# MarineRoboticsGroup/score

Hardware: AMD Instinct MI355X
Metric: socp_iters_per_sec (higher is better)
Workload: dtype f64; 1 GPU; BASELINE configs[3]: manhattan RA-SLAM, 20 robots x 1000 poses, 4 beacons, SOCP relaxation, 1 trial(s)/GPU, ADMM loop alone (polish off) to eps 1e-07; n=146995, m=80979, nnz_P=946147, parallelism=independent x1

## Files before the change

score_amd/csrc/score_hip.hip:

```cpp
#include <hip/hip_runtime.h>
#include <sched.h>
#include <sys/prctl.h>
#include <time.h>
#include <hip/hip_ext.h>

#include <cstdio>
#include <cstring>
#include <malloc.h>
#include <mutex>
#include <string>
#include <memory>
#include <optional>
#include <vector>

#include "score_driver.hpp"
#include <future>
#include "score_assemble.hpp"
#include "score_gn_kernels.hpp"
#include "score_round.hpp"
#include "score_kernels.hpp"
#include "score_polish.hpp"
#include "score_polish_device.hpp"
#include "score_setup_device.hpp"
#include "score_prec_wave.hpp"
// ... 766 lines not shown
    DevBuf<double> cone_vals;
    DevBuf<int32_t> node_col, diag_cols, prec_part_ptr;
    DevBuf<PrecWork> prec_work, factor_work;
    DevBuf<int64_t> q_entpart;
    int64_t q_ent_max = 0;
    static constexpr int64_t kHelpEntries = (int64_t)kPrecThreads * kPrecChunk;
    int n_help = 0;
    DevBuf<int32_t> vb_first, vb_end, vb_prob;
    int n_vblocks = 0;
    DevBuf<double> xtu, xy, s, r, z, p, p2, w, kx, step;
    DevBuf<double> pw_part, rz_part0, rz_part1, rz_meas0, rz_meas1, pres_part, dres_part;
    struct GenSource {
        const int32_t* rel_base; const int32_t* rel_to; const double* rel_t; const double* rel_R; const double* rel_kappa; const double* rel_tau;
        const int32_t* rng_a; const int32_t* rng_b; const double* rng_dist; const double* rng_prec;
    };
    const GenSource* gen_src = nullptr;
    int n_join_items = 0, n_join_chains = 0, n_join_seps = 0;
    DevBuf<JoinChain> join_jc;
    DevBuf<JoinItem> join_items;
    DevBuf<int32_t> join_sep_col, join_sep_diag, join_pcol, join_pprev, join_zero;
    DevBuf<double> join_rhs, join_tmp_p, join_tmp_rz, join_zb;
    DevBuf<int32_t> deep_map;
    bool prec_reg = false;
    size_t prec_reg_lds = 0;
    PolishData Q;
    std::future<void> polish_build;
    bool polish_on_device = false;
    bool derive_ag = false;
    int64_t hm_nnz = 0;
    CsrBufs Hm;
    struct PrecSet {
        const CsrBufs& mat;
        const BandBufs& band;
        const DevBuf<PrecWork>& fac_work;
        PrecSet(const CsrBufs& m, const BandBufs& b, const DevBuf<PrecWork>& fw) : mat(m), band(b), fac_work(fw) {}
        DevBuf<ChainDesc> chains;
        DevBuf<ChainLevelDesc> levels;
        DevBuf<PrecRecord> rec;
        DevBuf<int64_t> fac_range;
        DevBuf<double> fac, dinv;
        DevBuf<float> fac32;
        DevBuf<float> deep;
        size_t fac_doubles = 0;
        int64_t deep_floats = 0;
        bool use_fac32 = false;
        bool use_owner = false;
        DevBuf<int32_t> posd, poss, diagpos;
        DevBuf<int32_t> blk_part;
        int blocks() const { return band.on ? band.nblocks : mat.nblocks; }
        DevBuf<double> join_W, join_data;
        DevBuf<int32_t> join_posd, join_poss;
        bool link_on = false;
        DevBuf<int32_t> link_pcol, link_pshift, link_pos, link_status;
        DevBuf<double> link_Qt, link_Zr;
    };
    PrecSet pset[2] = {{K, Kb, factor_work}, {Hm, Hb, prec_work}};
    PrecSet &Kset = pset[0], &Hset = pset[1];
    enum class PrecDepth { chain, join, all };
    DevBuf<double> q_Pon, q_ccoef, q_Bbuf, q_fpart, q_X0, q_X1, q_g, q_delta, q_work, q_dummy, q_gd, q_pw;
    DevBuf<double> q_aabs, q_ck, q_theta, q_xstar;
    DevBuf<int32_t> q_cptr, q_ccone, q_cab, q_head, q_ishead, q_long, q_long_prob;
    int n_long = 0;
    DevBuf<int32_t> q_skip, q_reref, q_fskip, q_act;
    DevBuf<double> q_step;
    DevBuf<int64_t> q_seg_begin, q_seg_end;
    static constexpr int kFlagSlots = 32;
    char* h_ring = nullptr;
    size_t ring_slot_bytes = 0;
    int flag_slot = 0, ring_used = 0;
// ... 999 lines not shown
        const size_t deep_esz = h.bs >= 4 ? sizeof(float) : sizeof(double);
        for (const auto& ch : h.chains) {
            const ChainLevelDesc* lv = &h.levels[ch.level_begin];
            int64_t deep = 0;
            if (ch.n_levels >= 2) {
                const ChainLevelDesc& Lz = lv[ch.n_levels - 1];
                deep = Lz.offB + (int64_t)2 * h.bs * h.bs * Lz.N - lv[1].offR;
            }
            const int ng = std::max(8 * h.bs * h.bs, 32);
            if (ch.col_stride == 0 || ch.n_levels > kRecLevels || lv[0].nruns > kPreRunLanes || (ch.n_levels >= 2 && lv[1].N > kPrecThreads - kPreRunLanes) || (int64_t)ch.N * h.bs > (int64_t)pre_chunk * kPrecThreads ||
                deep > (int64_t)ng * (kPrecThreads - kPreRunLanes))
                pl.pre = false;
            const ChainLevelDesc& Lend = lv[ch.n_levels - 1];
            const size_t vec_bytes = (16 + (size_t)Lend.lds_off + (size_t)Lend.N * h.bs + 1 + (size_t)(lv[0].nruns + 1) * h.bs) * sizeof(double);
            lds_pre = std::max(lds_pre, vec_bytes + (((size_t)deep + 1) & ~(size_t)1) * deep_esz);
            lds_reg = std::max(lds_reg, vec_bytes);
        }
        if (lds_pre > 158 * 1024) pl.pre = false;
        pl.pre_lds = pl.pre ? lds_pre : 0;
        pl.reg = pl.pre && h.deep_ok && h.bs <= 3 && st.fac_fp32 != 0;
        pl.reg_lds = pl.reg ? lds_reg : 0;
        return pl;
    }
    void plan_chain_kernel(const HostSystem& h) {
        const ChainKernelPlan pl = chain_kernel_plan(h);
        prec_lds0 = pl.lds0; prec_lds = pl.lds;
        prec_pre = pl.pre; prec_pre_lds = pl.pre_lds;
        prec_reg = pl.reg; prec_reg_lds = pl.reg_lds;
        if (prec_reg) deep_map.upload(h.deep_map);
        const bool fallback = !prec_pre || (h.bs >= 4 && st.fac_fp32 == 0);
        if (fallback && prec_lds > 144 * 1024) throw std::runtime_error("chain too long: more than 129 segments of 1023 nodes (132 k) for the segmented chain solver, and beyond what the streaming kernel keeps in LDS");
        if (n_prec_chains(h)) with_bs([&](auto bs) { allow_big_lds<decltype(bs)::value>(); });
    }
    void adopt_band_view(HostSystem& h, PhaseTimer& pt) {
        if (band_job.valid()) {
            Kb.upload(band_job.get());
            if (Kb.on)
                for (int p = 0; p < h.count; ++p) h.kkt_bytes[(size_t)p] = Kb.L.bytes[(size_t)p] + 16.0 * (double)(h.xoff[p + 1] - h.xoff[p]);
            if (st.verbose)
                std::fprintf(stderr, "[score setup] band view of K: %s (%d band + %d csr + %d diag tiles, %d slots per row)\n", Kb.on ? "on" : "off",
                             Kb.L.n_band, Kb.L.n_csr, Kb.L.n_diag, Kb.L.S);
            pt.mark("band view of K (wait + upload)");
        }
        Kset.blk_part.upload(Kb.on ? Kb.L.part_ptr : h.rbK.part_ptr);
    }
    void carve_iterates(const HostSystem& h) {
        const size_t nm = (size_t)(h.n_tot + h.m_tot), nn = (size_t)h.n_tot, mm = (size_t)h.m_tot, cc = (size_t)h.count;
        const size_t kb = (size_t)Kset.blocks(), np_ = (size_t)n_prec;
        struct Piece { DevBuf<double>& buf; size_t count; Region<double> at; };
        Piece pieces[] = {{xtu, nm}, {xy, nm}, {s, mm}, {r, nn}, {z, nn}, {p, nn}, {p2, nn}, {w, nn}, {kx, nn}, {step, cc},
                          {pw_part, kb}, {rz_part0, np_}, {rz_part1, np_}, {rz_meas0, np_}, {rz_meas1, np_}};
// ... 498 lines not shown
    }

    hipEvent_t* tev = nullptr;
    std::shared_ptr<NewtonProbe> probe;
    template <class Kern, class... Args>
    void launch_on_stream(Kern kernel, dim3 grid, dim3 block, size_t lds_bytes, int slot, Args... args) {
        if (tev && slot >= 0)
            hipExtLaunchKernelGGL(kernel, grid, block, (unsigned)lds_bytes, stream, tev[2 * slot], tev[2 * slot + 1], 0, args...);
        else
            hipLaunchKernelGGL(kernel, grid, block, lds_bytes, stream, args...);
    }

    template <int MODE>
    void launch_prec(const PrecSet& S, const PrecArgs& pa, int slot = -1, PrecDepth depth = PrecDepth::all) {
        if (n_prec == 0) return;
        if (split.active) {
            if (pa.n_vec > 1) throw std::runtime_error("internal: several right-hand sides through the split chain kernel");
            WaveArgs wa{};
            wa.p = pa;
            wa.p.work = split_work.d;
            wa.items = split_items.d; wa.plans = split_plans.d; wa.stage_rel = split_stage.d;
            wa.xbuf = split_xbuf.d; wa.xflag = split_xflag.d; wa.epoch = split_epoch.d; wa.poll_limit = split_poll_limit;
            launch_on_stream(k_prec_wave<MODE>, dim3(n_prec), dim3(kWaveThreads), split_lds, slot, wa);
        } else with_bs([&](auto bs) { launch_prec_bs<decltype(bs)::value, MODE>(pa, slot, S.use_fac32); });
        if (pa.debug_skip) return;
        if (n_join_items && depth >= PrecDepth::join) join_apply<MODE>(S, pa);
        if (n_link_items && S.link_on && depth == PrecDepth::all) link_apply<MODE>(S, pa);
    }
    template <int BS, int MODE>
    void launch_prec_bs(const PrecArgs& pa_in, int slot, bool use_fac32) {
        PrecArgs pa = pa_in;
        const bool help = MODE == PREC_STEP && n_help > 0 && pa.rec != nullptr && !pa.debug_skip;
        const int n_prec = this->n_prec + (help ? n_help : 0);
        pa.split_update = (help && MODE == PREC_STEP) ? 1 : 0;
        const unsigned nv = (MODE == PREC_INIT && pa.n_vec > 1) ? (unsigned)pa.n_vec : 1u;
        if (nv == 1) pa.n_vec = 0;
        if constexpr (BS <= 3) {
            if (prec_reg && use_fac32) {
                launch_on_stream((k_prec_pre<BS, MODE, float, true>), dim3(n_prec, nv), dim3(kPrecThreads), prec_reg_lds, slot, pa);
                return;
            }
        }
        if (prec_pre && use_fac32) {
            launch_on_stream((k_prec_pre<BS, MODE, float>), dim3(n_prec, nv), dim3(kPrecThreads), prec_pre_lds, slot, pa);
            return;
        }
        if constexpr (BS <= 3) {
            if (prec_pre) {
                launch_on_stream((k_prec_pre<BS, MODE, double>), dim3(n_prec, nv), dim3(kPrecThreads), prec_pre_lds, slot, pa);
                return;
            }
        }
        pa.split_update = 0;
        if (prec_lds0) launch_on_stream((k_prec<BS, 3, MODE, true>), dim3(this->n_prec, nv), dim3(kPrecThreads), prec_lds, slot, pa);
        else launch_on_stream((k_prec<BS, 3, MODE, false>), dim3(this->n_prec, nv), dim3(kPrecThreads), prec_lds, slot, pa);
    }

    template <int BS>
    void allow_big_lds() {
        constexpr int kCeil = 158 * 1024;
        HIP_CHECK(hipFuncSetAttribute((const void*)k_prec<BS, 3, PREC_INIT, true>, hipFuncAttributeMaxDynamicSharedMemorySize, kCeil));
        HIP_CHECK(hipFuncSetAttribute((const void*)k_prec<BS, 3, PREC_STEP, true>, hipFuncAttributeMaxDynamicSharedMemorySize, kCeil));
        HIP_CHECK(hipFuncSetAttribute((const void*)k_prec<BS, 3, PREC_INIT, false>, hipFuncAttributeMaxDynamicSharedMemorySize, kCeil));
        HIP_CHECK(hipFuncSetAttribute((const void*)k_prec<BS, 3, PREC_STEP, false>, hipFuncAttributeMaxDynamicSharedMemorySize, kCeil));
        if constexpr (BS <= 3) {
            HIP_CHECK(hipFuncSetAttribute((const void*)k_prec_pre<BS, PREC_INIT, float, true>, hipFuncAttributeMaxDynamicSharedMemorySize, kCeil));
            HIP_CHECK(hipFuncSetAttribute((const void*)k_prec_pre<BS, PREC_STEP, float, true>, hipFuncAttributeMaxDynamicSharedMemorySize, kCeil));
            HIP_CHECK(hipFuncSetAttribute((const void*)k_prec_pre<BS, PREC_INIT, double>, hipFuncAttributeMaxDynamicSharedMemorySize, kCeil));
            HIP_CHECK(hipFuncSetAttribute((const void*)k_prec_pre<BS, PREC_STEP, double>, hipFuncAttributeMaxDynamicSharedMemorySize, kCeil));
        }
        HIP_CHECK(hipFuncSetAttribute((const void*)k_prec_pre<BS, PREC_INIT, float>, hipFuncAttributeMaxDynamicSharedMemorySize, kCeil));
        HIP_CHECK(hipFuncSetAttribute((const void*)k_prec_pre<BS, PREC_STEP, float>, hipFuncAttributeMaxDynamicSharedMemorySize, kCeil));
    }

    static unsigned xcd_grid_of(int n, int& chunk) {
        chunk = n >= 16 ? (n + 7) / 8 : 0;
        return chunk ? 8u * (unsigned)chunk : (unsigned)n;
    }
    unsigned xcd_grid(SpmvArgs& a, int nblocks) const {
        a.n_tiles = nblocks;
        return xcd_grid_of(nblocks, a.xcd_chunk);
    }
    UniRanges uni_for(int kblocks) const {
        UniRanges u{};
        u.on = (H->count == 1 && active_part_ptr.size() == 2) ? 1 : 0;
        u.l0 = 0; u.l1 = u.on ? active_part_ptr[1] : 0;
        u.k0 = 0; u.k1 = kblocks;
        return u;
    }
    template <int MODE, int NR>
// ... 2238 lines not shown
```

score_amd/csrc/score_host.hpp:

```cpp
#pragma once

#include <algorithm>
#include <atomic>
#include <cmath>
#include <chrono>
#include <cstdint>
#include <cstdio>
#include <cstring>
#include <numeric>
#include <stdexcept>
#include <string>
#include <thread>
#include <condition_variable>
#include <functional>
#include <mutex>

#include <pthread.h>
#include <sched.h>
#include <sys/resource.h>
#include <vector>

#include "../../include/score_hip.h"

namespace score {
// ... 617 lines not shown
    auto put = [&](int slot, int dt, int64_t idx) { map[(size_t)slot * lanes + dt] = (int32_t)(idx - fac_base); };
    for (size_t l = 1; l < lv.size(); ++l) {
        const ChainLevelDesc& L = lv[l];
        const bool last = (L.p == 0);
        for (int j = 0; j < L.nruns; ++j) {
            const int lo = last ? 0 : j * L.p;
            const int hi = last ? L.N : std::min(j * L.p + L.p - 1, L.N);
            const int len = std::max(hi - lo, 1);
            for (int q = 0; q < RMAX; ++q)
                for (int slot = 0; slot < 2; ++slot)
                    for (int e = 0; e < b2; ++e)
                        put(2 * b2 + (slot * RMAX + q) * b2 + e, L.lane0 + j,
                            L.offR + ((int64_t)(slot * b2 + e) * L.P + std::min(q, len - 1)) * L.nruns + j);
        }
        for (int j = 0; j < L.nsep; ++j)
            for (int slot = 0; slot < 2; ++slot)
                for (int e = 0; e < b2; ++e) put(2 * b2 + (2 * RMAX + slot) * b2 + e, L.lane0 + j, L.offS + (int64_t)(slot * b2 + e) * L.nsep + j);
        if (!last)
            for (int i = 0; i < L.N; ++i)
                for (int e = 0; e < 2 * b2; ++e) put((l == 1 ? 0 : 10 * b2) + e, L.lane0 + i, L.offB + (int64_t)e * L.N + i);
    }
}

inline void chain_solve_host(const ChainDesc& ch, const ChainLevelDesc* levels, const double* fac,
                             const int32_t* node_col, int bs, const double* r, double* z, double* scr) {
    const int b2 = bs * bs;
    const int32_t* nc = node_col + ch.node_begin;
    for (int lvl = 0; lvl < ch.n_levels; ++lvl) {
        const ChainLevelDesc& L = levels[ch.level_begin + lvl];
        const bool last = (L.p == 0);
        const int nsep = L.nsep;
        auto Rb = [&](int slot, int e, int q, int j) { return fac[L.offR + ((size_t)(slot * b2 + e) * L.P + q) * L.nruns + j]; };
        auto Sb = [&](int slot, int e, int j) { return fac[L.offS + (size_t)(slot * b2 + e) * nsep + j]; };
        auto in = [&](int i, int c) { return lvl == 0 ? r[nc[i] + c] : scr[(size_t)(L.vec_off + i) * bs + c]; };
        auto out = [&](int i, int c) -> double& {
            return lvl == 0 ? z[nc[i] + c] : scr[(size_t)(L.vec_off + i) * bs + c];
        };
        for (int j = 0; j < L.nruns; ++j) {
            const int lo = last ? 0 : j * L.p;
            const int hi = last ? L.N : std::min(j * L.p + L.p - 1, L.N);
            if (lo >= hi) continue;
            double prev[kMaxBs], cur[kMaxBs];
            for (int i = lo; i < hi; ++i) {
                for (int c = 0; c < bs; ++c) cur[c] = in(i, c);
                if (i > lo)
                    for (int c = 0; c < bs; ++c)
// ... 1102 lines not shown
```

score_amd/csrc/score_inspect.hpp:

```cpp
#pragma once

struct NewtonProbe {
    static constexpr int kCap = 1024;
    bool armed = false;
    std::vector<hipEvent_t> ev;
    struct Slot { int kind, step; bool real; };
    std::vector<Slot> slots;
    size_t marked = 0;
    double out[8] = {0, 0, 0, 0, 0, 0, 0, 0};
};
int probe_slot(HipBackend& be, int kind, int step) {
    NewtonProbe* np = be.probe.get();
    if (!np || !np->armed || (int)np->slots.size() >= NewtonProbe::kCap) return -1;
    np->slots.push_back(NewtonProbe::Slot{kind, step, false});
    be.tev = np->ev.data();
    return (int)np->slots.size() - 1;
}
void probe_mark(HipBackend& be, int used) {
    NewtonProbe* np = be.probe.get();
    if (!np) return;
    for (; np->marked < np->slots.size(); ++np->marked)
        if (np->slots[np->marked].step < used) np->slots[np->marked].real = true;
}
void probe_collect(HipBackend& be) {
// ... 186 lines not shown
}
int64_t get_polish_prec_of_negg(HipBackend& be, double* out, int64_t len) {
    if (!be.Q.available) return -1;
    if (out && len > 0) {
        PrecArgs pa = be.prec_args(be.Hset);
        pa.done = be.q_skip.d;
        be.prec_vectors(pa, be.r.d, be.q_negg.d, be.z.d, be.p.d, be.w.d, be.q_delta.d, be.q_dummy.d, be.q_pw.d);
        pa.rz_in = nullptr; pa.rz_out = be.rz_part0.d;
        be.launch_prec<PREC_INIT>(be.Hset, pa);
    }
    return read_row(be, DebugRow{"z", DebugRow::DevF64, be.z.d, be.H->n_tot}, out, len);
}
int64_t chain_map(HipBackend& be, bool by_chain, double* out, int64_t len) {
    const HostSystem& h = *be.H;
    std::vector<double> tmp(h.n_tot, -1.0);
    for (size_t ci = 0; ci < h.chains.size(); ++ci)
        for (int i = 0; i < h.chains[ci].N; ++i)
            for (int c = 0; c < h.bs; ++c) tmp[h.node_col[h.chains[ci].node_begin + i] + c] = by_chain ? (double)ci : (double)(h.chains[ci].node_begin + i);
    return copy_out_min(tmp.data(), (int64_t)tmp.size(), out, len);
}
int64_t get_chain_of_col(HipBackend& be, double* out, int64_t len) { return be.Q.available ? chain_map(be, false, out, len) : -1; }
int64_t get_chain_id_of_col(HipBackend& be, double* out, int64_t len) { return chain_map(be, true, out, len); }

int64_t get_vec(HipBackend& be, const char* name, double* out, int64_t len) {
    const HostSystem& h = *be.H;
    const std::string nm(name);
    using R = DebugRow;
    const bool ds = h.device_setup, polish = be.Q.available;
    const int64_t n = h.n_tot, m = h.m_tot, nk = (int64_t)h.K.col.size(), na = h.A.ptr.empty() ? 0 : (int64_t)h.A.ptr[(size_t)m];
    const int64_t n1 = ds ? be.g1_nnz : (int64_t)h.G1.col.size(), n2 = h.G2.ptr.empty() ? 0 : (int64_t)h.G2.ptr[(size_t)n];
    const PolishData& Q = be.Q;
    const R rows[] = {
        {"xt", R::DevF64, be.xtu.d, n}, {"u", R::DevF64, be.xtu.d + n, m},
        {"x", R::DevF64, be.xy.d, n}, {"y", R::DevF64, be.xy.d + n, m}, {"s", R::DevF64, be.s.d, m},
        {"r", R::DevF64, be.r.d, n}, {"z", R::DevF64, be.z.d, n},
        {"p", R::DevF64, be.dbg_p ? be.dbg_p : ((be.cg_iters % 2 == 1) ? be.p.d : be.p2.d), n},
        {"w", R::DevF64, be.w.d, n}, {"kx", R::DevF64, be.kx.d, n},
        {"D", ds ? R::DevF64 : R::HostF64, ds ? (const void*)be.Dd.d : h.D.data(), n},
        {"E", ds ? R::DevF64 : R::HostF64, ds ? (const void*)be.Ed.d : h.E.data(), m},
        {"K0", R::DevF64, be.K0d.d, nk}, {"K1", R::DevF64, be.K1d.d, nk}, {"Kval", R::DevF64, be.K.val.d, nk},
        {"Aval", R::DevF64, be.A_val.d, na}, {"G1val", R::DevF64, be.G1.val.d, n1}, {"G2val", R::DevF64, be.G2.val.d, n2},
        {"qs", R::DevF64, be.q.d, n}, {"bs", R::DevF64, be.b.d, m},
        {"invD", R::DevF64, be.invD.d, n}, {"invE", R::DevF64, be.invE.d, m},
        {"fac", R::DevF64, be.Kset.fac.d, (int64_t)be.Kset.fac_doubles},
        {"polish_g", R::DevF64, be.q_g.d, polish ? n : 0}, {"Hval", R::DevF64, be.Hm.val.d, polish ? be.hm_nnz : 0},
        {"Acol", R::DevI32, be.A_col.d, na}, {"Aptr", R::DevI32, be.A_ptr.d, m + 1},
        {"G1col", R::DevI32, be.G1.col.d, n1}, {"G1ptr", R::DevI32, be.G1.ptr.d, n + 1},
        {"G2col", R::DevI32, be.G2.col.d, n2}, {"G2ptr", R::DevI32, be.G2.ptr.d, n + 1}, {"G2split", R::DevI32, be.G2.split.d, n},
        {"Kcol_dev", R::DevI32, be.K.col.d, nk}, {"Kptr_dev", R::DevI32, be.K.ptr.d, n + 1},
        {"Kcol", R::HostI32, h.K.col.data(), nk}, {"Kptr", R::HostI32, h.K.ptr.data(), (int64_t)h.K.ptr.size()},
        {"is_head", ds ? R::DevI32 : R::HostI32, ds ? (const void*)be.q_ishead.d : Q.is_head.data(), ds ? n : (int64_t)Q.is_head.size(), polish},
        {"Hcol", be.polish_on_device ? R::DevI32 : R::HostI32, be.polish_on_device ? (const void*)be.Hm.col.d : Q.Hm.col.data(),
         be.polish_on_device ? be.hm_nnz : (int64_t)Q.Hm.col.size(), polish},
        {"Hptr", R::HostI32, Q.Hm.ptr.data(), (int64_t)Q.Hm.ptr.size(), polish},
        {"link_pairs", R::HostI32, be.link_plan.pair_cols.data(), be.n_link_items ? (int64_t)be.link_plan.pair_cols.size() : 0},
    };
    for (const R& r : rows)
        if (nm == r.name) return read_row(be, r, out, len);
    struct Computed { const char* name; int64_t (*fn)(HipBackend&, double*, int64_t); };
    static const Computed computed[] = {
        {"setup_scalars", get_setup_scalars}, {"device_setup", get_device_setup}, {"rep", get_rep}, {"links", get_links},
        {"newton_probe_arm", probe_arm}, {"newton_probe", get_newton_probe}, {"ag_device_check", get_ag_device_check},
        {"polish_build_check", get_polish_build_check}, {"polish_assemble_at_x", get_polish_assemble_at_x},
        {"polish_prec_of_negg", get_polish_prec_of_negg},
        {"chain_of_col", get_chain_of_col}, {"chain_id_of_col", get_chain_id_of_col}, {"matrix_source", get_matrix_source},
    };
    for (const Computed& c : computed)
        if (nm == c.name) return c.fn(be, out, len);
    return -1;
}

struct TimeAllActive {
    HipBackend& be;
    std::vector<int32_t> keep;
    explicit TimeAllActive(HipBackend& b) : be(b), keep((size_t)b.H->count) {
        const std::vector<int32_t> zero(keep.size(), 0);
        HIP_CHECK(sync_stream(be.stream));
        HIP_CHECK(hipMemcpyAsync(keep.data(), be.done.d, keep.size() * sizeof(int32_t), hipMemcpyDeviceToHost, be.stream));
        HIP_CHECK(sync_stream(be.stream));
        HIP_CHECK(hipMemcpyAsync(be.done.d, zero.data(), zero.size() * sizeof(int32_t), hipMemcpyHostToDevice, be.stream));
        HIP_CHECK(sync_stream(be.stream));
    }
    ~TimeAllActive() {
        (void)hipMemcpyAsync(be.done.d, keep.data(), keep.size() * sizeof(int32_t), hipMemcpyHostToDevice, be.stream);
        (void)sync_stream(be.stream);
    }
};
template <class F>
double time_launches(HipBackend& be, int warmup, int reps, F&& launch) {
    for (int i = 0; i < warmup; ++i) launch();
    HIP_CHECK(sync_stream(be.stream));
    HIP_CHECK(hipEventRecord(be.ev0, be.stream));
    for (int i = 0; i < reps; ++i) launch();
    HIP_CHECK(hipEventRecord(be.ev1, be.stream));
    HIP_CHECK(hipEventSynchronize(be.ev1));
    float t = 0;
    HIP_CHECK(hipEventElapsedTime(&t, be.ev0, be.ev1));
    return (double)t / std::max(1, reps);
}

void time_kernel(HipBackend& be, const std::string& which, int reps, double* ms) {
    PrecArgs pa = be.prec_args(be.Kset);
    pa.done = be.done.d;
    be.prec_vectors(pa, be.r.d, be.r.d, be.z.d, be.p.d, be.w.d, be.xtu.d, be.kx.d, be.pw_part.d);
    pa.rz_in = be.rz_part0.d; pa.rz_out = be.rz_part1.d;
    const VecArgs va = be.xupdate_args(be.p.d, be.rz_part0.d, 1);
    const dim3 blk(kThreads);
    auto once = [&]() {
        if (which == "rhs") { SpmvArgs ra = be.spmv_args(be.G1, be.xtu.d); ra.apply_update = 1; be.launch_spmv<MODE_RHS>(be.G1, ra); }
        else if (which.rfind("prec_init:", 0) == 0) { pa.debug_skip = std::atoi(which.c_str() + 10); be.launch_prec<PREC_INIT>(be.Kset, pa); }
// ... 98 lines not shown
```

score_amd/csrc/score_kernels.hpp:

```cpp
#pragma once

#include <type_traits>

#include <hip/hip_runtime.h>

#include "score_host.hpp"
#include "score_band.hpp"

namespace score {

#ifdef SCORE_NT_STORES
#define NTS(lhs, val) __builtin_nontemporal_store((val), &(lhs))
#else
#define NTS(lhs, val) ((lhs) = (val))
#endif
#if defined(SCORE_NT_STORES) || defined(SCORE_NT_PREC)
#define NTSP(lhs, val) __builtin_nontemporal_store((val), &(lhs))
#else
#define NTSP(lhs, val) ((lhs) = (val))
#endif

constexpr int kThreads = 256;
constexpr int kUnroll = kTileNnz / kThreads;
constexpr int kLongUnroll = 2;
// ... 828 lines not shown
        const int end_ptr = (t == 0) ? meta.w : 0;
        if (NR > 1 && rs > 0) spmv_tile<MODE, NR, UNR>(a, b, meta, prob, end_ptr, rs, prod, red, srow, h.lg, h.dn0);
        else spmv_tile<MODE, 1, UNR>(a, b, meta, prob, end_ptr, 0, prod, red, srow, h.lg, h.dn0);
    }
}
template <int MODE, int NR, int NP, bool LDSW = false>
__global__ __launch_bounds__(kThreads) void k_spmv_band(SpmvArgs a) { spmv_band_body<MODE, NR, NP, LDSW>(a); }

__global__ __launch_bounds__(kThreads) void k_band_pack(const int32_t* __restrict__ dst, const double* __restrict__ val, double* __restrict__ V, int64_t nnz) {
    const int64_t k = (int64_t)blockIdx.x * kThreads + threadIdx.x;
    if (k >= nnz) return;
    const int d = dst[k];
    if (d >= 0) V[d] = val[k];
}

constexpr int kRecLevels = 7;
struct alignas(16) PrecRecord {
    PrecWork wk;
    ChainDesc ch;
    int32_t pad_;
    ChainLevelDesc lv[kRecLevels];
};
static_assert(sizeof(PrecRecord) == 512, "PrecRecord is read as 32 int4");

struct PrecArgs {
    const PrecWork* work;
    const PrecRecord* rec;
    const ChainDesc* chains;
    const ChainLevelDesc* levels;
    const double* fac;
    const float* fac32;
    const float* deep;
    const int32_t* node_col;
    const int32_t* diag_cols;
    const double* dinv;
    const int32_t* done;
    const int32_t* prec_part_ptr;
    const int32_t* kblk_part_ptr;
    UniRanges uni;
    double* r;
    double* z;
    double* p;
    const double* w;
    double* xt;
    double* kx;
    const double* rz_in;
// ... 435 lines not shown
}

__device__ __forceinline__ void lds_barrier() {
    __builtin_amdgcn_fence(__ATOMIC_RELEASE, "workgroup", "local");
    __builtin_amdgcn_s_barrier();
    __builtin_amdgcn_fence(__ATOMIC_ACQUIRE, "workgroup", "local");
}

constexpr int kPreRunLanes = 256;
template <int BS>
struct PreTile {
    static constexpr int B2 = BS * BS;
    static constexpr int NG = (8 * B2 > 32) ? 8 * B2 : 32;
    static constexpr int CH = (BS >= 4) ? 8 : kPrecChunk;
};

template <int BS, int MODE, typename FT, bool REGDEEP>
__device__ __forceinline__ void prec_pre_body(const PrecArgs& a);
template <int BS, int MODE, typename FT = double, bool REGDEEP = false>
__global__ __launch_bounds__(kPrecThreads) void k_prec_pre(PrecArgs a) {
    if (MODE == PREC_INIT) prec_select_vector(a);
    prec_pre_body<BS, MODE, FT, REGDEEP>(a);
}
template <int BS, int MODE, typename FT, bool REGDEEP>
__device__ __forceinline__ void prec_pre_body(const PrecArgs& a) {
    static_assert(!REGDEEP || (sizeof(FT) == 4 && BS <= 3), "register-resident coarse levels: 4-byte stream, blocks up to 3 x 3");
    KernelStamp stamp(a.tstamp);
    constexpr int RMAX = 3;
    constexpr int B2 = BS * BS;
    constexpr int oRun = REGDEEP ? 2 * B2 : 0;
    constexpr int oBk2 = 10 * B2;
    constexpr int NG = REGDEEP ? 12 * B2 : PreTile<BS>::NG;
    constexpr int oCl = oRun + 2 * RMAX * B2, oCr = oCl + B2;
    constexpr int kStageLanes = kPrecThreads - kPreRunLanes;
    constexpr int CH = PreTile<BS>::CH;
    using LT = typename std::conditional<(BS >= 4 || REGDEEP), FT, double>::type;
    extern __shared__ __attribute__((aligned(16))) double lds[];
    __shared__ PrecRecord srec;
    double* red = lds;
    const int t = threadIdx.x;
    double acc_rz = 0.0, acc_pw = 0.0;
    int4 rec4 = make_int4(0, 0, 0, 0);
    if (t < 32) rec4 = reinterpret_cast<const int4*>(a.rec + blockIdx.x)[t];
    const int dn0 = a.uni.on ? a.done[0] : 0;
    if (MODE == PREC_STEP && a.uni.on) {
        const int i0 = a.uni.l0 + t, j0 = a.uni.k0 + t;
        if (i0 < a.uni.l1) acc_rz = a.rz_in[i0];
        if (j0 < a.uni.k1) acc_pw = a.pw_part[j0];
        for (int i = i0 + kPrecThreads; i < a.uni.l1; i += kPrecThreads) acc_rz += a.rz_in[i];
        for (int i = j0 + kPrecThreads; i < a.uni.k1; i += kPrecThreads) acc_pw += a.pw_part[i];
    }
    if (t < 32) reinterpret_cast<int4*>(&srec)[t] = rec4;
    __syncthreads();
    const PrecWork wk = srec.wk;
    const ChainLevelDesc* sLv = srec.lv;
    const int prob = wk.prob;
    const int dn_ld = a.uni.on ? dn0 : a.done[prob];
    int bl0 = 0, bl1 = 0, bk0 = 0, bk1 = 0;
    if (MODE == PREC_STEP && !a.uni.on) {
        bl0 = a.prec_part_ptr[prob]; bl1 = a.prec_part_ptr[prob + 1];
        bk0 = a.kblk_part_ptr[prob]; bk1 = a.kblk_part_ptr[prob + 1];
    }
    int dn = 0;
    if (a.early_done) {
        dn = dn_ld;
        if (dn) return;
    }
    const int dn_late = a.early_done ? 0 : dn_ld;
    if (MODE == PREC_INIT && a.gate_init && threadIdx.x == 0 && (int)blockIdx.x == a.prec_part_ptr[prob]) {
        a.gate_init[prob] = a.early_done ? dn : dn_late;
        a.gate_used[prob] = 0;
    }
    if (MODE == PREC_STEP && !a.uni.on) {
        const int l0 = bl0, l1 = bl1, k0 = bk0, k1 = bk1;
        if (l0 + t < l1) acc_rz = a.rz_in[l0 + t];
        if (k0 + t < k1) acc_pw = a.pw_part[k0 + t];
        for (int i = l0 + t + kPrecThreads; i < l1; i += kPrecThreads) acc_rz += a.rz_in[i];
        for (int i = k0 + t + kPrecThreads; i < k1; i += kPrecThreads) acc_pw += a.pw_part[i];
// ... 10 lines not shown
        for (int u = 0; u < kPrecChunk; ++u) {
            idx[u] = min(wk.index + t + u * kPrecThreads, e_end - 1);
            pv[u] = a.p[idx[u]]; wv[u] = a.w[idx[u]]; xv[u] = a.xt_zero ? 0.0 : a.xt[idx[u]]; kv[u] = a.kx[idx[u]];
        }
        block_sum2_n<kPrecWaves>(acc_rz, acc_pw, red);
        const double alpha = acc_pw > 0.0 ? acc_rz / acc_pw : 0.0;
        if (a.gate_flag && (a.gate_first ? !(acc_rz > 0.0) : !(acc_rz > gref))) return;
#pragma unroll
        for (int u = 0; u < kPrecChunk; ++u) {
            if (wk.index + t + u * kPrecThreads < e_end) {
                NTSP(a.xt[idx[u]], xv[u] + alpha * pv[u]);
                NTSP(a.kx[idx[u]], kv[u] + alpha * wv[u]);
            }
        }
        return;
    }
    if (wk.kind == 1) {
        if (dn || dn_late) return;
        bool stop;
        local = prec_jacobi_item<MODE>(a, wk, acc_rz, acc_pw, red, stop);
        if (stop) return;
    } else {
        const double gref = (MODE == PREC_STEP && a.gate_flag && !a.gate_first) ? a.gate_ref[prob] : 0.0;
        const ChainDesc ch = srec.ch;
        const FT* __restrict__ fac = sizeof(FT) == 4 ? (const FT*)(const void*)a.fac32 : (const FT*)(const void*)a.fac;
        const int N = ch.N;
        const int NB = N * BS;
        const int nl = ch.n_levels;
        const int stride = ch.col_stride, col0 = ch.col0;
        auto colof = [&](int node) -> int { return col0 + node * stride; };
        double* vb = lds + 16;
        double* v0 = vb;
        const ChainLevelDesc L0 = sLv[0];
        const ChainLevelDesc Lz = sLv[nl - 1];
        LT* lfac = reinterpret_cast<LT*>(vb + Lz.lds_off + Lz.N * BS + 1);
        auto pad = [](const ChainLevelDesc& L, int i) -> int { return (int)(((uint32_t)i * L.inv_p) >> 20); };
        auto nodep = [&](const ChainLevelDesc& L, int i) -> double* { return vb + L.lds_off + i * BS + pad(L, i); };
        int64_t deep_base = 0;
        int deep_cnt = 0;
        if (nl >= 2) {
            deep_base = sLv[1].offR;
            deep_cnt = (int)(Lz.offB + (int64_t)2 * B2 * Lz.N - deep_base);
        }
        double* xch = REGDEEP ? vb + Lz.lds_off + Lz.N * BS + 1 : reinterpret_cast<double*>(lfac + ((deep_cnt + 1) & ~1));
        int cols[CH];
        double rv[CH], wv[CH];
#pragma unroll
        for (int u = 0; u < CH; ++u) {
            const int idx = min(t + u * kPrecThreads, NB - 1);
            const int node = idx / BS;
            cols[u] = colof(node) + (idx - node * BS);
        }
        constexpr bool kLateW = (BS >= 4);
#pragma unroll
        for (int u = 0; u < CH; ++u) {
            rv[u] = a.r_in[cols[u]];
            if (MODE == PREC_STEP && !kLateW) wv[u] = a.w[cols[u]];
        }
        FT Gr[NG];
        const bool l0_last = (L0.p == 0);
        if (t < kPreRunLanes) {
            if ((t & ~63) < L0.nruns && !(a.debug_skip & 1)) {
                const int j = min(t, L0.nruns - 1);
                const int lo = l0_last ? 0 : j * L0.p;
// ... 148 lines not shown
            const int len = hi - lo;
            const int jpad = l0_last ? 0 : j;
            if (len > 0) {
                double y[RMAX][BS];
#pragma unroll
                for (int q = 0; q < RMAX; ++q) {
                    const double* src = v0 + (lo + min(q, len - 1)) * BS + jpad;
#pragma unroll
                    for (int c = 0; c < BS; ++c) y[q][c] = src[c];
                }
                run_solve0(y, len);
#pragma unroll
                for (int q = 0; q < RMAX; ++q) {
                    if (q < len) {
                        double* dst = v0 + (lo + q) * BS + jpad;
#pragma unroll
                        for (int c = 0; c < BS; ++c) dst[c] = y[q][c];
                    }
                }
            }
        }
        lds_barrier();
        if (nl >= 2 && !dbg_nophase) {
            const ChainLevelDesc L1 = sLv[1];
            if (t < L0.nsep) {
                const int s = t * L0.p + L0.p - 1;
                const bool has_r = (s + 1 < L0.N);
                const double* pv_ = v0 + s * BS + t;
                const double* pm = v0 + (s - 1) * BS + t;
                const double* pp = has_r ? v0 + (s + 1) * BS + t + 1 : pv_;
                double v[BS], ym[BS], yp[BS];
#pragma unroll
                for (int c = 0; c < BS; ++c) { v[c] = pv_[c]; ym[c] = pm[c]; yp[c] = pp[c]; }
#pragma unroll
                for (int c = 0; c < BS; ++c) {
                    double acc = v[c];
#pragma unroll
                    for (int k = 0; k < BS; ++k) acc -= G[oCl + c * BS + k] * ym[k] + G[oCr + c * BS + k] * yp[k];
                    nodep(L1, t)[c] = acc;
                }
            }
            lds_barrier();
        }
        constexpr int kHalf = CH / 2;
        double pv[kHalf], wq[kHalf], xv[kHalf], kv[kHalf];
        auto upd_load = [&](auto half) {
            constexpr int u0 = decltype(half)::value * kHalf;
#pragma unroll
            for (int u = 0; u < kHalf; ++u) {
                pv[u] = a.p[cols[u0 + u]]; wq[u] = a.w[cols[u0 + u]]; xv[u] = a.xt_zero ? 0.0 : a.xt[cols[u0 + u]]; kv[u] = a.kx[cols[u0 + u]];
            }
        };
        auto upd_store = [&](auto half) {
            constexpr int u0 = decltype(half)::value * kHalf;
#pragma unroll
            for (int u = 0; u < kHalf; ++u) {
                if (t + (u0 + u) * kPrecThreads < NB) {
                    NTSP(a.xt[cols[u0 + u]], xv[u] + alpha * pv[u]);
                    NTSP(a.kx[cols[u0 + u]], kv[u] + alpha * wq[u]);
                }
            }
        };
        using H0 = std::integral_constant<int, 0>;
        using H1 = std::integral_constant<int, 1>;
        constexpr bool kLateUpdate = (BS >= 4);
        const bool own_update = (MODE == PREC_STEP) && !a.split_update;
        if (own_update && !kLateUpdate) upd_load(H0());
        const int dt = t - kPreRunLanes;
        for (int l = 1; l < nl && !dbg_nophase; ++l) {
            const ChainLevelDesc L = sLv[l];
            const bool last = (L.p == 0);
            const int dl = REGDEEP ? dt - L.lane0 : dt;
            if (dt >= 0 && dl >= 0 && dl < L.nruns) {
                const int j = dl;
                const int lo = last ? 0 : j * L.p;
                const int hi = last ? L.N : min(j * L.p + L.p - 1, L.N);
                const int len = hi - lo;
                if (len > 0) {
                    if (!REGDEEP) {
                        const int eP = L.P * L.nruns;
                        const LT* R = lfac + (L.offR - deep_base);
#pragma unroll
                        for (int q = 0; q < RMAX; ++q) {
                            const LT* Rq = R + min(q, len - 1) * L.nruns + j;
#pragma unroll
                            for (int e = 0; e < B2; ++e) {
                                G[q * B2 + e] = Rq[e * eP];
                                G[(RMAX + q) * B2 + e] = Rq[(B2 + e) * eP];
                            }
                        }
                    }
                    double* vr = vb + L.lds_off + lo * BS + (last ? 0 : j);
                    double y[RMAX][BS];
#pragma unroll
                    for (int q = 0; q < RMAX; ++q)
#pragma unroll
                        for (int c = 0; c < BS; ++c) y[q][c] = vr[min(q, len - 1) * BS + c];
                    run_solve0(y, len);
#pragma unroll
                    for (int q = 0; q < RMAX; ++q) {
                        if (q < len) {
#pragma unroll
                            for (int c = 0; c < BS; ++c) vr[q * BS + c] = y[q][c];
                        }
                    }
                }
            }
            lds_barrier();
            if (last) break;
            const ChainLevelDesc Ln = sLv[l + 1];
            if (dt >= 0 && dl >= 0 && dl < L.nsep) {
                const int js = dl;
                if (!REGDEEP) {
                    const LT* S = lfac + (L.offS - deep_base);
#pragma unroll
                    for (int e = 0; e < B2; ++e) {
                        G[oCl + e] = S[e * L.nsep + js];
                        G[oCr + e] = S[(B2 + e) * L.nsep + js];
                    }
                }
                const int s = js * L.p + L.p - 1;
                const bool has_r = (s + 1 < L.N);
                const double* pv_ = vb + L.lds_off + s * BS + js;
                const double* pm = vb + L.lds_off + (s - 1) * BS + js;
                const double* pp = has_r ? vb + L.lds_off + (s + 1) * BS + js + 1 : pv_;
                double v[BS], ym[BS], yp[BS];
#pragma unroll
                for (int c = 0; c < BS; ++c) { v[c] = pv_[c]; ym[c] = pm[c]; yp[c] = pp[c]; }
                double* dst = nodep(Ln, js);
#pragma unroll
                for (int c = 0; c < BS; ++c) {
                    double acc = v[c];
#pragma unroll
                    for (int k = 0; k < BS; ++k) acc -= G[oCl + c * BS + k] * ym[k] + G[oCr + c * BS + k] * yp[k];
                    dst[c] = acc;
                }
            }
            lds_barrier();
        }
        for (int l = nl - 2; l >= 1 && !dbg_nophase; --l) {
            const ChainLevelDesc Lb = sLv[l];
            const ChainLevelDesc Ln = sLv[l + 1];
            const int db = REGDEEP ? dt - Lb.lane0 : dt;
            if (dt >= 0 && db >= 0 && db < Lb.N) {
                const int i = db;
                LT Vw[2 * B2];
                if (REGDEEP) {
#pragma unroll
                    for (int e = 0; e < 2 * B2; ++e) Vw[e] = (l == 1) ? G[e] : G[oBk2 + e];
                } else {
                    const LT* Bk = lfac + (Lb.offB - deep_base);
#pragma unroll
                    for (int e = 0; e < 2 * B2; ++e) Vw[e] = Bk[e * Lb.N + i];
                }
                const int nsep = Lb.nsep;
                const int j = pad(Lb, i);
                const bool is_sep = (i - j * Lb.p == Lb.p - 1) && (j < nsep);
                const int jl = max(j - 1, 0), jr = min(j, max(nsep - 1, 0));
                double* pvx = vb + Lb.lds_off + i * BS + j;
                const double* pul = nodep(Ln, jl);
                const double* pur = nodep(Ln, jr);
                double v[BS], ul[BS], ur[BS];
#pragma unroll
                for (int c = 0; c < BS; ++c) { v[c] = pvx[c]; ul[c] = pul[c]; ur[c] = pur[c]; }
#pragma unroll
                for (int c = 0; c < BS; ++c) {
                    double acc = v[c];
#pragma unroll
                    for (int k = 0; k < BS; ++k) acc -= Vw[c * BS + k] * ul[k] + Vw[B2 + c * BS + k] * ur[k];
                    pvx[c] = is_sep ? ur[c] : acc;
                }
            }
            lds_barrier();
        }
        if (own_update && !kLateUpdate) { upd_store(H0()); upd_load(H1()); }
        if (nl >= 2 && !dbg_nophase) {
            const ChainLevelDesc L1 = sLv[1];
            const int nsep = L0.nsep;
            double c_last[BS];
#pragma unroll
            for (int c = 0; c < BS; ++c) c_last[c] = 0.0;
            if (t < nsep) {
                const int s = t * L0.p + L0.p - 1;
                double xs[BS];
#pragma unroll
                for (int c = 0; c < BS; ++c) xs[c] = nodep(L1, t)[c];
#pragma unroll
                for (int c = 0; c < BS; ++c) {
                    double sl = 0.0, sr = 0.0;
#pragma unroll
                    for (int k = 0; k < BS; ++k) { sl += G[oCl + k * BS + c] * xs[k]; sr += G[oCr + k * BS + c] * xs[k]; }
                    c_last[c] = sl;
                    xch[(size_t)(t + 1) * BS + c] = sr;
                    v0[s * BS + t + c] = xs[c];
                }
            }
            lds_barrier();
            if (t < L0.nruns) {
                const int lo = t * L0.p;
                const int hi = min(t * L0.p + L0.p - 1, L0.N);
// ... 486 lines not shown
```

Measured before the change: 17710 iters/s.

## Add uniform-chain preconditioner kernel deriving chain geometry from block index

```diff
diff --git a/score_amd/csrc/score_hip.hip b/score_amd/csrc/score_hip.hip
--- a/score_amd/csrc/score_hip.hip
+++ b/score_amd/csrc/score_hip.hip
@@ -812,6 +812,7 @@
     DevBuf<double> join_rhs, join_tmp_p, join_tmp_rz, join_zb;
     DevBuf<int32_t> deep_map;
     bool prec_reg = false;
+    bool uni_off = false;
     size_t prec_reg_lds = 0;
     PolishData Q;
     std::future<void> polish_build;
@@ -835,6 +836,7 @@
         int64_t deep_floats = 0;
         bool use_fac32 = false;
         bool use_owner = false;
+        UniPlan uni{};
         DevBuf<int32_t> posd, poss, diagpos;
         DevBuf<int32_t> blk_part;
         int blocks() const { return band.on ? band.nblocks : mat.nblocks; }
@@ -1880,11 +1882,19 @@
         pl.reg_lds = pl.reg ? lds_reg : 0;
         return pl;
     }
+    UniPlan uni_plan(const HostSystem& h, const std::vector<ChainDesc>& cs, const std::vector<ChainLevelDesc>& ls) const {
+        return uniform_chain_plan(h.prec_work, h.prec_part_ptr, cs, ls, std::max(1, h.rep), (int)h.prec_work.size() + n_help);
+    }
     void plan_chain_kernel(const HostSystem& h) {
         const ChainKernelPlan pl = chain_kernel_plan(h);
         prec_lds0 = pl.lds0; prec_lds = pl.lds;
         prec_pre = pl.pre; prec_pre_lds = pl.pre_lds;
         prec_reg = pl.reg; prec_reg_lds = pl.reg_lds;
+        if (prec_reg && !split.active) {
+            Kset.uni = uni_plan(h, h.chains, h.levels);
+            Hset.uni = (h.rep > 1 && st.polish) ? uni_plan(h, h.chainsH, h.levelsH) : Kset.uni;
+        }
+        if (st.verbose) std::fprintf(stderr, "[score setup] chain sets uniform (k_prec_uni): K %d, Newton %d\n", Kset.uni.on, Hset.uni.on);
         if (prec_reg) deep_map.upload(h.deep_map);
         const bool fallback = !prec_pre || (h.bs >= 4 && st.fac_fp32 == 0);
         if (fallback && prec_lds > 144 * 1024) throw std::runtime_error("chain too long: more than 129 segments of 1023 nodes (132 k) for the segmented chain solver, and beyond what the streaming kernel keeps in LDS");
@@ -2429,13 +2439,14 @@
             wa.items = split_items.d; wa.plans = split_plans.d; wa.stage_rel = split_stage.d;
             wa.xbuf = split_xbuf.d; wa.xflag = split_xflag.d; wa.epoch = split_epoch.d; wa.poll_limit = split_poll_limit;
             launch_on_stream(k_prec_wave<MODE>, dim3(n_prec), dim3(kWaveThreads), split_lds, slot, wa);
-        } else with_bs([&](auto bs) { launch_prec_bs<decltype(bs)::value, MODE>(pa, slot, S.use_fac32); });
+        } else with_bs([&](auto bs) { launch_prec_bs<decltype(bs)::value, MODE>(S, pa, slot); });
         if (pa.debug_skip) return;
         if (n_join_items && depth >= PrecDepth::join) join_apply<MODE>(S, pa);
         if (n_link_items && S.link_on && depth == PrecDepth::all) link_apply<MODE>(S, pa);
     }
     template <int BS, int MODE>
-    void launch_prec_bs(const PrecArgs& pa_in, int slot, bool use_fac32) {
+    void launch_prec_bs(const PrecSet& S, const PrecArgs& pa_in, int slot) {
+        const bool use_fac32 = S.use_fac32;
         PrecArgs pa = pa_in;
         const bool help = MODE == PREC_STEP && n_help > 0 && pa.rec != nullptr && !pa.debug_skip;
         const int n_prec = this->n_prec + (help ? n_help : 0);
@@ -2444,6 +2455,10 @@
         if (nv == 1) pa.n_vec = 0;
         if constexpr (BS <= 3) {
             if (prec_reg && use_fac32) {
+                if (S.uni.on && !uni_off && pa.rec != nullptr) {
+                    launch_on_stream((k_prec_uni<BS, MODE>), dim3(n_prec, nv), dim3(kPrecThreads), prec_reg_lds, slot, pa, S.uni);
+                    return;
+                }
                 launch_on_stream((k_prec_pre<BS, MODE, float, true>), dim3(n_prec, nv), dim3(kPrecThreads), prec_reg_lds, slot, pa);
                 return;
             }
@@ -2473,6 +2488,8 @@
         if constexpr (BS <= 3) {
             HIP_CHECK(hipFuncSetAttribute((const void*)k_prec_pre<BS, PREC_INIT, float, true>, hipFuncAttributeMaxDynamicSharedMemorySize, kCeil));
             HIP_CHECK(hipFuncSetAttribute((const void*)k_prec_pre<BS, PREC_STEP, float, true>, hipFuncAttributeMaxDynamicSharedMemorySize, kCeil));
+            HIP_CHECK(hipFuncSetAttribute((const void*)k_prec_uni<BS, PREC_INIT>, hipFuncAttributeMaxDynamicSharedMemorySize, kCeil));
+            HIP_CHECK(hipFuncSetAttribute((const void*)k_prec_uni<BS, PREC_STEP>, hipFuncAttributeMaxDynamicSharedMemorySize, kCeil));
             HIP_CHECK(hipFuncSetAttribute((const void*)k_prec_pre<BS, PREC_INIT, double>, hipFuncAttributeMaxDynamicSharedMemorySize, kCeil));
             HIP_CHECK(hipFuncSetAttribute((const void*)k_prec_pre<BS, PREC_STEP, double>, hipFuncAttributeMaxDynamicSharedMemorySize, kCeil));
         }
diff --git a/score_amd/csrc/score_host.hpp b/score_amd/csrc/score_host.hpp
--- a/score_amd/csrc/score_host.hpp
+++ b/score_amd/csrc/score_host.hpp
@@ -663,6 +663,105 @@
     }
 }
 
+constexpr int kUniLevels = 7;
+struct UniLevel {
+    int32_t N, p, nruns, P, nsep, lds_off;
+    uint32_t inv_p;
+    int32_t lane0;
+};
+struct UniGeom {
+    int32_t N, n_levels, mask, pad_;
+    int64_t offS_rel;
+    int32_t col0[4], deep[4];
+    int64_t fac[4];
+    UniLevel lv[kUniLevels];
+};
+struct UniPlan {
+    int32_t on;
+    int32_t n_items, ipp, nchain, per_rep;
+    int32_t n_first;
+    uint32_t ipp_inv, per_rep_inv;
+    int32_t col_stride;
+    UniGeom g[2];
+};
+
+inline UniPlan uniform_chain_plan(const std::vector<PrecWork>& work, const std::vector<int32_t>& part_ptr, const std::vector<ChainDesc>& cs,
+                                  const std::vector<ChainLevelDesc>& ls, int rep, int n_launch) {
+    UniPlan up{};
+    const UniPlan none{};
+    const int count = (int)part_ptr.size() - 1;
+    if (count < 1 || cs.empty() || work.empty() || part_ptr[0] != 0 || part_ptr[(size_t)count] != (int32_t)work.size()) return none;
+    const int ipp = part_ptr[1] - part_ptr[0];
+    int nchain = 0;
+    while (nchain < ipp && work[(size_t)nchain].kind == 0) ++nchain;
+    if (nchain == 0 || rep < 1 || nchain % rep) return none;
+    const int per_rep = nchain / rep;
+    for (int q = 0; q < count; ++q) {
+        if (part_ptr[(size_t)q + 1] - part_ptr[(size_t)q] != ipp) return none;
+        for (int i = 0; i < ipp; ++i) {
+            const PrecWork& w = work[(size_t)part_ptr[(size_t)q] + i];
+            if ((w.kind == 0) != (i < nchain) || w.prob != q) return none;
+            if (w.kind == 0 && (w.index < 0 || (size_t)w.index >= cs.size())) return none;
+        }
+    }
+    auto chain = [&](int q, int k, int c) -> const ChainDesc& { return cs[(size_t)work[(size_t)part_ptr[(size_t)q] + k * per_rep + c].index]; };
+    up.n_items = (int32_t)work.size(); up.ipp = ipp; up.nchain = nchain; up.per_rep = per_rep;
+    up.ipp_inv = (1u << 20) / (uint32_t)ipp + 1; up.per_rep_inv = (1u << 20) / (uint32_t)per_rep + 1;
+    for (int w = 0; w < std::max(n_launch, (int)work.size()); ++w)
+        if ((int)(((uint64_t)w * up.ipp_inv) >> 20) != w / ipp) return none;
+    for (int i = 0; i < ipp; ++i)
+        if ((int)(((uint64_t)i * up.per_rep_inv) >> 20) != i / per_rep) return none;
+    up.col_stride = chain(0, 0, 0).col_stride;
+    if (up.col_stride == 0) return none;
+    int n_first = 1;
+    while (n_first < per_rep && chain(0, 0, n_first).N == chain(0, 0, 0).N) ++n_first;
+    up.n_first = n_first;
+    auto quantities = [&](const ChainDesc& ch, int64_t (&x)[3]) { x[0] = ch.col0; x[1] = ch.deep_off; x[2] = ls[(size_t)ch.level_begin].offR; };
+    auto fits32 = [](int64_t v) { return v >= INT32_MIN && v <= INT32_MAX; };
+    for (int g = 0; g < 2; ++g) {
+        const int c_lo = g == 0 ? 0 : n_first, c_hi = g == 0 ? n_first : per_rep;
+        if (c_lo >= c_hi) { up.g[g] = up.g[0]; continue; }
+        UniGeom& G = up.g[g];
+        const ChainDesc& c0 = chain(0, 0, c_lo);
+        if (c0.n_levels < 1 || c0.n_levels > kUniLevels || c0.deep_map_off < 0) return none;
+        const ChainLevelDesc* l0 = &ls[(size_t)c0.level_begin];
+        if (c0.n_levels >= 2 && l0[1].lane0 < 0) return none;
+        G.N = c0.N; G.n_levels = c0.n_levels; G.mask = l0[0].pad_; G.offS_rel = l0[0].offS - l0[0].offR;
+        for (int l = 0; l < c0.n_levels; ++l)
+            G.lv[l] = UniLevel{l0[l].N, l0[l].p, l0[l].nruns, l0[l].P, l0[l].nsep, l0[l].lds_off, l0[l].inv_p, l0[l].lane0};
+        int64_t x0[3], xq[3] = {0, 0, 0}, xk[3] = {0, 0, 0}, xc[3] = {0, 0, 0}, x[3];
+        quantities(c0, x0);
+        if (count > 1) { quantities(chain(1, 0, c_lo), x); for (int j = 0; j < 3; ++j) xq[j] = x[j] - x0[j]; }
+        if (rep > 1) { quantities(chain(0, 1, c_lo), x); for (int j = 0; j < 3; ++j) xk[j] = x[j] - x0[j]; }
+        if (c_lo + 1 < c_hi) { quantities(chain(0, 0, c_lo + 1), x); for (int j = 0; j < 3; ++j) xc[j] = x[j] - x0[j]; }
+        for (int j = 0; j < 3; ++j) x0[j] -= c_lo * xc[j];
+        for (int j = 0; j < 2; ++j)
+            if (!fits32(x0[j]) || !fits32(xq[j]) || !fits32(xk[j]) || !fits32(xc[j])) return none;
+        for (int q = 0; q < count; ++q)
+            for (int k = 0; k < rep; ++k)
+                for (int c = c_lo; c < c_hi; ++c) {
+                    const ChainDesc& ch = chain(q, k, c);
+                    if (ch.N != c0.N || ch.n_levels != c0.n_levels || ch.col_stride != up.col_stride || ch.prob != q || ch.deep_map_off < 0) return none;
+                    const ChainLevelDesc* lv = &ls[(size_t)ch.level_begin];
+                    if (lv[0].pad_ != l0[0].pad_ || lv[0].offS - lv[0].offR != G.offS_rel) return none;
+                    for (int l = 0; l < c0.n_levels; ++l)
+                        if (lv[l].N != l0[l].N || lv[l].p != l0[l].p || lv[l].nruns != l0[l].nruns || lv[l].P != l0[l].P || lv[l].nsep != l0[l].nsep ||
+                            lv[l].lds_off != l0[l].lds_off || lv[l].inv_p != l0[l].inv_p || lv[l].lane0 != l0[l].lane0)
+                            return none;
+                    quantities(ch, x);
+                    for (int j = 0; j < 3; ++j) {
+                        const int64_t want = x0[j] + q * xq[j] + k * xk[j] + c * xc[j];
+                        if (x[j] != want || (j < 2 && !fits32(want))) return none;
+                    }
+                }
+        G.col0[0] = (int32_t)x0[0]; G.col0[1] = (int32_t)xq[0]; G.col0[2] = (int32_t)xk[0]; G.col0[3] = (int32_t)xc[0];
+        G.deep[0] = (int32_t)x0[1]; G.deep[1] = (int32_t)xq[1]; G.deep[2] = (int32_t)xk[1]; G.deep[3] = (int32_t)xc[1];
+        G.fac[0] = x0[2]; G.fac[1] = xq[2]; G.fac[2] = xk[2]; G.fac[3] = xc[2];
+    }
+    up.on = 1;
+    return up;
+}
+
 inline void chain_solve_host(const ChainDesc& ch, const ChainLevelDesc* levels, const double* fac,
                              const int32_t* node_col, int bs, const double* r, double* z, double* scr) {
     const int b2 = bs * bs;
diff --git a/score_amd/csrc/score_inspect.hpp b/score_amd/csrc/score_inspect.hpp
--- a/score_amd/csrc/score_inspect.hpp
+++ b/score_amd/csrc/score_inspect.hpp
@@ -232,6 +232,7 @@
 int64_t get_chain_of_col(HipBackend& be, double* out, int64_t len) { return be.Q.available ? chain_map(be, false, out, len) : -1; }
 int64_t get_chain_id_of_col(HipBackend& be, double* out, int64_t len) { return chain_map(be, true, out, len); }
 
+int64_t get_uniform_chain_check(HipBackend& be, double* out, int64_t len);
 int64_t get_vec(HipBackend& be, const char* name, double* out, int64_t len) {
     const HostSystem& h = *be.H;
     const std::string nm(name);
@@ -274,6 +275,7 @@
         {"polish_build_check", get_polish_build_check}, {"polish_assemble_at_x", get_polish_assemble_at_x},
         {"polish_prec_of_negg", get_polish_prec_of_negg},
         {"chain_of_col", get_chain_of_col}, {"chain_id_of_col", get_chain_id_of_col}, {"matrix_source", get_matrix_source},
+        {"uniform_chain_check", get_uniform_chain_check},
     };
     for (const Computed& c : computed)
         if (nm == c.name) return c.fn(be, out, len);
@@ -296,6 +298,36 @@
         (void)sync_stream(be.stream);
     }
 };
+void uniform_chain_check_set(HipBackend& be, const HipBackend::PrecSet& S, const double* r_in, bool ready, double* out) {
+    const bool eligible = ready && S.uni.on && be.prec_reg && S.use_fac32 && !be.split.active && be.H->bs <= 3;
+    out[0] = 0.0; out[1] = 0.0; out[2] = eligible ? 1.0 : 0.0;
+    if (!eligible) return;
+    const size_t n = (size_t)be.H->n_tot, np = (size_t)be.n_prec;
+    DevBuf<double> zs, ps, rz;
+    zs.alloc(2 * n); ps.alloc(2 * n); rz.alloc(2 * np);
+    TimeAllActive all_active(be);
+    zs.zero(be.stream); ps.zero(be.stream); rz.zero(be.stream);
+    for (int v = 0; v < 2; ++v) {
+        PrecArgs pa = be.prec_args(S);
+        pa.done = be.done.d;
+        be.prec_vectors(pa, be.r.d, r_in, zs.d + v * n, ps.d + v * n, be.w.d, be.xtu.d, be.kx.d, be.pw_part.d);
+        pa.rz_in = nullptr; pa.rz_out = rz.d + v * np;
+        be.uni_off = (v == 0);
+        be.launch_prec<PREC_INIT>(S, pa, -1, HipBackend::PrecDepth::chain);
+        be.uni_off = false;
+    }
+    const std::vector<double> z = down_f64(be, zs.d, 2 * n), part = down_f64(be, rz.d, 2 * np);
+    for (size_t i = 0; i < n; ++i) out[0] += std::memcmp(&z[i], &z[n + i], sizeof(double)) != 0;
+    for (size_t i = 0; i < np; ++i) out[1] += std::memcmp(&part[i], &part[np + i], sizeof(double)) != 0;
+}
+int64_t get_uniform_chain_check(HipBackend& be, double* out, int64_t len) {
+    if (out && len >= 6) {
+        uniform_chain_check_set(be, be.Kset, be.r.d, true, out);
+        uniform_chain_check_set(be, be.Hset, be.q_negg.d, be.Q.available && be.q_negg.d != nullptr && be.Hset.fac.d != nullptr, out + 3);
+    }
+    return 6;
+}
+
 template <class F>
 double time_launches(HipBackend& be, int warmup, int reps, F&& launch) {
     for (int i = 0; i < warmup; ++i) launch();
diff --git a/score_amd/csrc/score_kernels.hpp b/score_amd/csrc/score_kernels.hpp
--- a/score_amd/csrc/score_kernels.hpp
+++ b/score_amd/csrc/score_kernels.hpp
@@ -874,6 +874,8 @@
     ChainLevelDesc lv[kRecLevels];
 };
 static_assert(sizeof(PrecRecord) == 512, "PrecRecord is read as 32 int4");
+
+static_assert(kUniLevels == kRecLevels, "UniPlan (score_host.hpp) carries a record's level table");
 
 struct PrecArgs {
     const PrecWork* work;
@@ -1355,8 +1357,21 @@
     if (MODE == PREC_INIT) prec_select_vector(a);
     prec_pre_body<BS, MODE, FT, REGDEEP>(a);
 }
+template <int BS, int MODE, typename FT, bool REGDEEP, bool UNI>
+__device__ __forceinline__ void prec_pre_impl(const PrecArgs& a, const UniPlan& up);
 template <int BS, int MODE, typename FT, bool REGDEEP>
 __device__ __forceinline__ void prec_pre_body(const PrecArgs& a) {
+    const UniPlan none{};
+    prec_pre_impl<BS, MODE, FT, REGDEEP, false>(a, none);
+}
+template <int BS, int MODE>
+__global__ __launch_bounds__(kPrecThreads) void k_prec_uni(PrecArgs a, const UniPlan up) {
+    if (MODE == PREC_INIT) prec_select_vector(a);
+    prec_pre_impl<BS, MODE, float, true, true>(a, up);
+}
+template <int BS, int MODE, typename FT, bool REGDEEP, bool UNI>
+__device__ __forceinline__ void prec_pre_impl(const PrecArgs& a, const UniPlan& up) {
+    static_assert(!UNI || REGDEEP, "uniform chain sets: the register-resident variant only");
     static_assert(!REGDEEP || (sizeof(FT) == 4 && BS <= 3), "register-resident coarse levels: 4-byte stream, blocks up to 3 x 3");
     KernelStamp stamp(a.tstamp);
     constexpr int RMAX = 3;
@@ -1373,8 +1388,24 @@
     double* red = lds;
     const int t = threadIdx.x;
     double acc_rz = 0.0, acc_pw = 0.0;
+    int uq = 0, ug = 0, ucol0 = 0, udeep = 0;
+    int64_t ufac = 0;
+    bool uni_chain = false;
+    if constexpr (UNI) {
+        const uint32_t w_ = blockIdx.x;
+        uq = (int)(((uint64_t)w_ * up.ipp_inv) >> 20);
+        const int i_ = (int)w_ - uq * up.ipp;
+        const int k_ = (int)(((uint64_t)(uint32_t)i_ * up.per_rep_inv) >> 20);
+        const int c_ = i_ - k_ * up.per_rep;
+        uni_chain = (int)w_ < up.n_items && i_ < up.nchain;
+        ug = c_ >= up.n_first ? 1 : 0;
+        const UniGeom& G_ = up.g[ug];
+        ucol0 = G_.col0[0] + uq * G_.col0[1] + k_ * G_.col0[2] + c_ * G_.col0[3];
+        udeep = G_.deep[0] + uq * G_.deep[1] + k_ * G_.deep[2] + c_ * G_.deep[3];
+        ufac = G_.fac[0] + uq * G_.fac[1] + k_ * G_.fac[2] + c_ * G_.fac[3];
+    }
     int4 rec4 = make_int4(0, 0, 0, 0);
-    if (t < 32) rec4 = reinterpret_cast<const int4*>(a.rec + blockIdx.x)[t];
+    if (!uni_chain && t < 32) rec4 = reinterpret_cast<const int4*>(a.rec + blockIdx.x)[t];
     const int dn0 = a.uni.on ? a.done[0] : 0;
     if (MODE == PREC_STEP && a.uni.on) {
         const int i0 = a.uni.l0 + t, j0 = a.uni.k0 + t;
@@ -1383,10 +1414,23 @@
         for (int i = i0 + kPrecThreads; i < a.uni.l1; i += kPrecThreads) acc_rz += a.rz_in[i];
         for (int i = j0 + kPrecThreads; i < a.uni.k1; i += kPrecThreads) acc_pw += a.pw_part[i];
     }
-    if (t < 32) reinterpret_cast<int4*>(&srec)[t] = rec4;
-    __syncthreads();
-    const PrecWork wk = srec.wk;
+    if (!uni_chain) {
+        if (t < 32) reinterpret_cast<int4*>(&srec)[t] = rec4;
+        __syncthreads();
+    }
+    const PrecWork wk = uni_chain ? PrecWork{0, 0, 0, uq} : srec.wk;
     const ChainLevelDesc* sLv = srec.lv;
+    auto lvl = [&](int l) -> ChainLevelDesc {
+        if constexpr (UNI) {
+            const UniLevel u = up.g[ug].lv[l];
+            ChainLevelDesc L;
+            L.N = u.N; L.p = u.p; L.nruns = u.nruns; L.P = u.P; L.nsep = u.nsep; L.vec_off = 0; L.lds_off = u.lds_off; L.inv_p = u.inv_p;
+            L.offR = ufac; L.offS = ufac + up.g[ug].offS_rel; L.offB = 0; L.lane0 = u.lane0; L.pad_ = up.g[ug].mask;
+            return L;
+        } else {
+            return sLv[l];
+        }
+    };
     const int prob = wk.prob;
     const int dn_ld = a.uni.on ? dn0 : a.done[prob];
     int bl0 = 0, bl1 = 0, bk0 = 0, bk1 = 0;
@@ -1443,7 +1487,13 @@
         if (stop) return;
     } else {
         const double gref = (MODE == PREC_STEP && a.gate_flag && !a.gate_first) ? a.gate_ref[prob] : 0.0;
-        const ChainDesc ch = srec.ch;
+        ChainDesc ch;
+        if constexpr (UNI) {
+            ch = ChainDesc{};
+            ch.N = up.g[ug].N; ch.n_levels = up.g[ug].n_levels; ch.col_stride = up.col_stride; ch.col0 = ucol0; ch.deep_off = udeep;
+        } else {
+            ch = srec.ch;
+        }
         const FT* __restrict__ fac = sizeof(FT) == 4 ? (const FT*)(const void*)a.fac32 : (const FT*)(const void*)a.fac;
         const int N = ch.N;
         const int NB = N * BS;
@@ -1452,15 +1502,15 @@
         auto colof = [&](int node) -> int { return col0 + node * stride; };
         double* vb = lds + 16;
         double* v0 = vb;
-        const ChainLevelDesc L0 = sLv[0];
-        const ChainLevelDesc Lz = sLv[nl - 1];
+        const ChainLevelDesc L0 = lvl(0);
+        const ChainLevelDesc Lz = lvl(nl - 1);
         LT* lfac = reinterpret_cast<LT*>(vb + Lz.lds_off + Lz.N * BS + 1);
         auto pad = [](const ChainLevelDesc& L, int i) -> int { return (int)(((uint32_t)i * L.inv_p) >> 20); };
         auto nodep = [&](const ChainLevelDesc& L, int i) -> double* { return vb + L.lds_off + i * BS + pad(L, i); };
         int64_t deep_base = 0;
         int deep_cnt = 0;
         if (nl >= 2) {
-            deep_base = sLv[1].offR;
+            deep_base = lvl(1).offR;
             deep_cnt = (int)(Lz.offB + (int64_t)2 * B2 * Lz.N - deep_base);
         }
         double* xch = REGDEEP ? vb + Lz.lds_off + Lz.N * BS + 1 : reinterpret_cast<double*>(lfac + ((deep_cnt + 1) & ~1));
@@ -1655,7 +1705,7 @@
         }
         lds_barrier();
         if (nl >= 2 && !dbg_nophase) {
-            const ChainLevelDesc L1 = sLv[1];
+            const ChainLevelDesc L1 = lvl(1);
             if (t < L0.nsep) {
                 const int s = t * L0.p + L0.p - 1;
                 const bool has_r = (s + 1 < L0.N);
@@ -1700,8 +1750,11 @@
         const bool own_update = (MODE == PREC_STEP) && !a.split_update;
         if (own_update && !kLateUpdate) upd_load(H0());
         const int dt = t - kPreRunLanes;
+        ChainLevelDesc Lfw{}, Lbb{}, Lbn{};
+        if constexpr (UNI) { Lfw = lvl(min(1, nl - 1)); Lbb = lvl(max(nl - 2, 0)); Lbn = Lz; }
         for (int l = 1; l < nl && !dbg_nophase; ++l) {
-            const ChainLevelDesc L = sLv[l];
+            ChainLevelDesc L;
+            if constexpr (UNI) { L = Lfw; Lfw = lvl(min(l + 1, nl - 1)); } else { L = lvl(l); }
             const bool last = (L.p == 0);
             const int dl = REGDEEP ? dt - L.lane0 : dt;
             if (dt >= 0 && dl >= 0 && dl < L.nruns) {
@@ -1741,7 +1794,8 @@
             }
             lds_barrier();
             if (last) break;
-            const ChainLevelDesc Ln = sLv[l + 1];
+            ChainLevelDesc Ln;
+            if constexpr (UNI) { Ln = Lfw; } else { Ln = lvl(l + 1); }
             if (dt >= 0 && dl >= 0 && dl < L.nsep) {
                 const int js = dl;
                 if (!REGDEEP) {
@@ -1772,8 +1826,8 @@
             lds_barrier();
         }
         for (int l = nl - 2; l >= 1 && !dbg_nophase; --l) {
-            const ChainLevelDesc Lb = sLv[l];
-            const ChainLevelDesc Ln = sLv[l + 1];
+            ChainLevelDesc Lb, Ln;
+            if constexpr (UNI) { Lb = Lbb; Ln = Lbn; Lbn = Lb; Lbb = lvl(max(l - 1, 0)); } else { Lb = lvl(l); Ln = lvl(l + 1); }
             const int db = REGDEEP ? dt - Lb.lane0 : dt;
             if (dt >= 0 && db >= 0 && db < Lb.N) {
                 const int i = db;
@@ -1808,7 +1862,7 @@
         }
         if (own_update && !kLateUpdate) { upd_store(H0()); upd_load(H1()); }
         if (nl >= 2 && !dbg_nophase) {
-            const ChainLevelDesc L1 = sLv[1];
+            const ChainLevelDesc L1 = lvl(1);
             const int nsep = L0.nsep;
             double c_last[BS];
 #pragma unroll
```

New measurement: 17460 iters/s. 0.986x the previous value.
